# vgteam/vg

Hardware: AMD Instinct MI355X
Metric: reads/sec aligned (150 bp) (higher is better)
Workload: dtype u16

## Files before the change

### vg_amd/csrc/backend_hip.hip

```cpp
#include <chrono>
#include <thread>
#include <hip/hip_runtime.h>
#include <cstdlib>
#include <string>
#include "backend.hpp"
#include "pack_hip.hpp"

namespace vgk {

static __device__ __forceinline__ uint32_t from_lane_above(uint32_t x) {
    return (uint32_t)__builtin_amdgcn_update_dpp(0, (int)x, 0x138 , 0xf, 0xf, true);
}

template <int K>
struct TbStage {
    static constexpr uint32_t REC = (K + 3) / 4, RB = REC - 4;
    static constexpr uint32_t DWORDS = TB_TILE * 64u * REC;
    uint32_t* lds;
    __device__ __forceinline__ uint32_t* slot_a(uint32_t t, uint32_t lane) const { const uint32_t s = t % TB_TILE; return lds + (s * 64u + (lane ^ s)) * 4u; }
    __device__ __forceinline__ uint32_t* slot_b(uint32_t t, uint32_t lane) const { return lds + TB_TILE * 64u * 4u + ((t % TB_TILE) * 64u + lane) * RB; }
    __device__ __forceinline__ void flush(uint32_t* tile, uint32_t lane) const {
        __builtin_amdgcn_fence(__ATOMIC_ACQ_REL, "wavefront");
        __builtin_amdgcn_wave_barrier();
#pragma unroll
// ... 43 lines not shown
#pragma unroll
        for (int d = 32; d > 0; d >>= 1) { const uint32_t o = (uint32_t)__shfl_xor((int)shortest, d, 64); shortest = o < shortest ? o : shortest; }
        steady_steps(wd.G, shortest, wd.n_steps, steady_from, steady_to);
        steady_from = (uint32_t)__builtin_amdgcn_readfirstlane((int)steady_from); steady_to = (uint32_t)__builtin_amdgcn_readfirstlane((int)steady_to);
    }
    if constexpr (!CODES) {
        uint32_t t = 0;
        for (; t < steady_from; ++t) {
            if ((t & 3u) == 0) lane_prefetch(s, P, t);
            const uint32_t rh = from_lane_above(s.out_h), rf = from_lane_above(s.out_f), ri = from_lane_above(s.info);
            lane_step<K, S8, false, KEY3>(s, P, t, rh, rf, ri, nullptr, nullptr);
        }
        for (; t < steady_to; ++t) {
            if ((t & 3u) == 0) lane_prefetch(s, P, t);
            const uint32_t rh = from_lane_above(s.out_h), rf = from_lane_above(s.out_f), ri = from_lane_above(s.info);
            lane_step<K, S8, false, KEY3, false, true>(s, P, t, rh, rf, ri, nullptr, nullptr);
        }
        for (; t < wd.n_steps; ++t) {
            if ((t & 3u) == 0) lane_prefetch(s, P, t);
            const uint32_t rh = from_lane_above(s.out_h), rf = from_lane_above(s.out_f), ri = from_lane_above(s.info);
            lane_step<K, S8, false, KEY3>(s, P, t, rh, rf, ri, nullptr, nullptr);
        }
    }
    for (uint32_t t = 0; CODES && t < wd.n_steps; ++t) {
        if ((t & 3u) == 0) lane_prefetch(s, P, t);
        const uint32_t rh = from_lane_above(s.out_h);
        const uint32_t rf = from_lane_above(s.out_f);
        const uint32_t ri = from_lane_above(s.info);
        if constexpr (!CODES) {
        } else if constexpr (REWALK) {
            lane_step<K, S8, false>(s, P, t, rh, rf, ri, nullptr, nullptr);
            if (tb) {
                uint32_t* st = stage_lds[threadIdx.x >> 6] + lane * (TB_BND_CHUNK * 2u);
                const uint32_t slot = (t ^ lane) & (TB_BND_CHUNK - 1u);
                *reinterpret_cast<uint2*>(st + slot * 2u) = make_uint2(s.out_h, s.out_f);
                if ((t & (TB_BND_CHUNK - 1u)) == TB_BND_CHUNK - 1u || t + 1u == wd.n_steps) {
                    __builtin_amdgcn_fence(__ATOMIC_ACQ_REL, "wavefront"); __builtin_amdgcn_wave_barrier();
                    uint4* out = reinterpret_cast<uint4*>(tb + tb_bnd(wd.tb_off, wd.n_steps, t & ~(TB_BND_CHUNK - 1u), lane));
#pragma unroll
                    for (uint32_t j = 0; j < TB_BND_CHUNK; j += 2) {
                        const uint2 a = *reinterpret_cast<const uint2*>(st + ((j ^ lane) & (TB_BND_CHUNK - 1u)) * 2u), b = *reinterpret_cast<const uint2*>(st + (((j + 1u) ^ lane) & (TB_BND_CHUNK - 1u)) * 2u);
                        out[j >> 1] = make_uint4(a.x, a.y, b.x, b.y);
                    }
                    __builtin_amdgcn_fence(__ATOMIC_ACQ_REL, "wavefront"); __builtin_amdgcn_wave_barrier();
                }
                lane_store_checkpoint<K>(s, P, wd, t, lane);
            }
        } else if constexpr (TB_TILE > 1) {
            lane_step<K, S8, true, false, NOKEY>(s, P, t, rh, rf, ri, tb ? stage.slot_a(t, lane) : nullptr, stage.slot_b(t, lane));
            if (tb && ((t % TB_TILE) == TB_TILE - 1u || t + 1u == wd.n_steps)) stage.flush(tb + tb_tile_base(wd.tb_off, t, REC), lane);
        } else
            lane_step<K, S8, true, false, NOKEY>(s, P, t, rh, rf, ri, tb ? tb + tb_dword(wd.tb_off, t, lane, REC, 0) : nullptr, tb ? tb + tb_dword(wd.tb_off, t, lane, REC, 4) : nullptr);
    }
    if constexpr (NOKEY) return;
    if (REWALK || !CODES || !P.fused) {
#pragma unroll
        for (int half = 0; half < 2; ++half) {
            uint32_t prob; unsigned long long key;
            if (lane_best(s, half, prob, key)) atomicMax(&P.best[prob], key);
        }
        return;
    }
    unsigned long long* mine = reinterpret_cast<unsigned long long*>(stage_lds[threadIdx.x >> 6]);
#pragma unroll
    for (int half = 0; half < 2; ++half) {
        uint32_t prob; unsigned long long key = 0;
        if (!lane_best(s, half, prob, key)) key = 0;
        mine[lane * 2 + half] = key;
    }
    __threadfence();
    const uint32_t n_slots = 2u * (64u / wd.G);
    for (uint32_t slot = lane; slot < n_slots; slot += 64u) {
        const uint32_t q = slot >> 1, half = slot & 1u;
        if (wd.first_pair + q >= wd.pair_end) continue;
        const uint32_t prob = P.order[2u * (wd.first_pair + q) + half];
        if (prob == 0xffffffffu) continue;
        unsigned long long key = 0;
        for (uint32_t g = 0; g < wd.G; ++g) { const unsigned long long k = mine[(q * wd.G + g) * 2 + half]; key = k > key ? k : key; }
        walk_one(P, prob, key);
    }
}

#ifndef VGK_WALK_WAVES
#define VGK_WALK_WAVES 0
#endif
#if VGK_WALK_WAVES
__global__ __launch_bounds__(256, VGK_WALK_WAVES) void gssw_walk_kernel(const GsswParams P, const int in_fill_order) {
#else
__global__ __launch_bounds__(256) void gssw_walk_kernel(const GsswParams P, const int in_fill_order) {
#endif
    const uint32_t k = blockIdx.x * blockDim.x + threadIdx.x;
    if (!in_fill_order) { if (k < P.n_problems) walk_one(P, k, P.best[k]); return; }
    if (k >= 2u * P.n_pairs) return;
    const uint32_t i = P.order[k];
    if (i != 0xffffffffu) walk_one(P, i, P.best[i]);
}
__global__ __launch_bounds__(64) void banded_geometry_kernel(const BGeomParams P) {
    const uint32_t i = blockIdx.x * blockDim.x + threadIdx.x;
    if (i < P.n) banded_geometry_one(P, i);
}

__global__ __launch_bounds__(64) void gssw_walk_first_kernel(const GsswParams P, const int in_fill_order) {
    __shared__ uint32_t blk[2 * WD_DWORDS * 64];
    __shared__ int16_t tab[WD_TAB];
    if (threadIdx.x < WD_TAB) tab[threadIdx.x] = wd_table_entry(P, threadIdx.x);
    __syncthreads();
    const uint32_t k = blockIdx.x * blockDim.x + threadIdx.x;
    if (!in_fill_order) { if (k < P.n_problems) walk_first_one(P, k, P.best[k], blk + threadIdx.x, 64, tab); return; }
    if (k >= 2u * P.n_pairs) return;
    const uint32_t i = P.order[k];
    if (i != 0xffffffffu) walk_first_one(P, i, P.best[i], blk + threadIdx.x, 64, tab);
}
__global__ __launch_bounds__(64) void gssw_refill_layout_kernel(const GsswParams P) {
    refill_layout_one(P, blockIdx.x * blockDim.x + threadIdx.x);
}
__global__ __launch_bounds__(256) void gssw_refill_restore_kernel(const GsswParams P) {
    const uint32_t i = blockIdx.x * blockDim.x + threadIdx.x;
    if (i < P.n_problems) refill_restore_one(P, i);
}
__global__ __launch_bounds__(256) void gssw_walk_missed_kernel(const GsswParams P) {
    const uint32_t k = blockIdx.x * blockDim.x + threadIdx.x;
    if (k >= *tb_miss_count(P)) return;
    const uint32_t i = tb_miss_list(P)[k];
    walk_one(P, i, P.best[i]);
}

template <int K, bool S8>
__global__ __launch_bounds__(256, 2) void gssw_band_kernel(const GsswParams P) {
    const uint32_t wave = P.wave_begin + blockIdx.x * 4u + (threadIdx.x >> 6);
    if (wave >= P.wave_begin + P.wave_count) return;
    band_fill_lane<K, S8>(P, P.waves[wave], threadIdx.x & 63u);
}
__global__ __launch_bounds__(256) void gssw_bandwalk_kernel(const GsswParams P) {
    const uint32_t k = blockIdx.x * blockDim.x + threadIdx.x;
    if (k >= 2u * P.n_pairs) return;
    const uint32_t i = P.order[k];
    if (i != 0xffffffffu) bandwalk_one(P, i, P.best[i]);
}
template <int K, bool S8>
__global__ __launch_bounds__(64, 2) void gssw_rewalk_kernel(const GsswParams P) {
    __shared__ uint32_t win[(TB_CKPT / 2) * ((K + 3) / 4) * 64];
    const uint32_t count = *tb_miss_count(P);
    const uint32_t* list = tb_miss_list(P);
    for (uint32_t k = blockIdx.x * 64u + threadIdx.x; k < count; k += gridDim.x * 64u) {
        const uint32_t i = list[k];
        rewalk_one<K, S8>(P, i, P.best[i], win + threadIdx.x, 64u);
    }
}

static __device__ __forceinline__ uint32_t ops_of(const vgk_result* res, uint32_t i, uint32_t n) {
    return (i < n && res[i].status == VGK_OK) ? res[i].n_ops : 0u;
}
__global__ __launch_bounds__(256) void ops_scan_kernel(const vgk_result* res, uint32_t n, uint32_t* offs, uint32_t* sums) {
    __shared__ uint32_t wave_total[4];
    const uint32_t i0 = (blockIdx.x * 256u + threadIdx.x) * 4u, lane = threadIdx.x & 63u, w = threadIdx.x >> 6;
    const uint32_t c0 = ops_of(res, i0, n), c1 = ops_of(res, i0 + 1, n), c2 = ops_of(res, i0 + 2, n), c3 = ops_of(res, i0 + 3, n);
    uint32_t incl = c0 + c1 + c2 + c3;
#pragma unroll
    for (uint32_t d = 1; d < 64; d <<= 1) { const uint32_t up = __shfl_up(incl, d, 64); if (lane >= d) incl += up; }
    if (lane == 63) wave_total[w] = incl;
    __syncthreads();
    uint32_t before = 0;
    for (uint32_t k = 0; k < w; ++k) before += wave_total[k];
    uint32_t at = before + incl - (c0 + c1 + c2 + c3);
// ... 886 lines not shown
        return hipMemsetAsync(dst, 0, bytes, stream) == hipSuccess ? VGK_OK : VGK_ENODEV;
    }
    int sync() override {
        hipSetDevice(dev);
        return hipStreamSynchronize(stream) == hipSuccess ? VGK_OK : VGK_ENODEV;
    }
    size_t win_tmp_bytes(uint32_t n, uint32_t n_waves_cap) override { hipSetDevice(dev); return hip_win_tmp_bytes(n, n_waves_cap); }
    int win_stage1(const WinParams& P, void* tmp, size_t tmp_bytes) override { hipSetDevice(dev); return hip_win_stage1(P, tmp, tmp_bytes, copy); }
    int win_stage2(const WinParams& P, void* tmp, size_t tmp_bytes) override { hipSetDevice(dev); return hip_win_stage2(P, tmp, tmp_bytes, copy); }
    int download_side(void* dst, const void* src, size_t bytes) override {
        hipSetDevice(dev);
        if (hipMemcpyAsync(dst, src, bytes, hipMemcpyDeviceToHost, copy) != hipSuccess) return VGK_ENODEV;
        return hipStreamSynchronize(copy) == hipSuccess ? VGK_OK : VGK_ENODEV;
    }
    int fill_side(void* dst, int byte, size_t bytes) override {
        hipSetDevice(dev);
        return hipMemsetAsync(dst, byte, bytes, copy) == hipSuccess ? VGK_OK : VGK_ENODEV;
    }
    template <int K> int launch_fill_k(const GsswParams& p, hipStream_t stream) {
        const dim3 grid((p.wave_count + 3) / 4), block(256);
        const bool s8 = p.scale == 8, re = p.tb_mode == TB_REWALK;
        if (p.spec_fill == 1) {
            if (s8 && p.key3) hipLaunchKernelGGL((gssw_fill_kernel<K, true, false, false, true>), grid, block, 0, stream, p);
            else if (s8) hipLaunchKernelGGL((gssw_fill_kernel<K, true, false, false>), grid, block, 0, stream, p); else hipLaunchKernelGGL((gssw_fill_kernel<K, false, false, false>), grid, block, 0, stream, p);
            return VGK_OK;
        }
        if (p.spec_fill == 2 && s8 && !re && !p.fused) { hipLaunchKernelGGL((gssw_fill_kernel<K, true, false, true, false, true>), grid, block, 0, stream, p); return VGK_OK; }
        if (re) { if (s8) hipLaunchKernelGGL((gssw_fill_kernel<K, true, true>), grid, block, 0, stream, p); else hipLaunchKernelGGL((gssw_fill_kernel<K, false, true>), grid, block, 0, stream, p); }
        else    { if (s8) hipLaunchKernelGGL((gssw_fill_kernel<K, true, false>), grid, block, 0, stream, p); else hipLaunchKernelGGL((gssw_fill_kernel<K, false, false>), grid, block, 0, stream, p); }
        return VGK_OK;
    }
    int launch_fill(const GsswParams& p, hipStream_t stream) {
        switch (p.K) {
            case 16: return launch_fill_k<16>(p, stream);
            case 19: return launch_fill_k<19>(p, stream);
            case 20: return launch_fill_k<20>(p, stream);
            case 24: return launch_fill_k<24>(p, stream);
            default: return VGK_EINVAL;
        }
    }
    template <int K> void launch_rewalk_k(const GsswParams& p, hipStream_t stream) {
        const dim3 grid(1024), block(64);
        if (p.scale == 8) hipLaunchKernelGGL((gssw_rewalk_kernel<K, true>), grid, block, 0, stream, p); else hipLaunchKernelGGL((gssw_rewalk_kernel<K, false>), grid, block, 0, stream, p);
    }
    template <int K> void launch_band_k(const GsswParams& p, hipStream_t stream) {
        const dim3 grid((p.wave_count + 3) / 4), block(256);
        if (p.scale == 8) hipLaunchKernelGGL((gssw_band_kernel<K, true>), grid, block, 0, stream, p); else hipLaunchKernelGGL((gssw_band_kernel<K, false>), grid, block, 0, stream, p);
    }
    void launch_walk(const GsswParams& p0, const FillLaunch* launches, uint32_t n, hipStream_t stream, int lane = 0) {
        sev_set[lane] = false;
        if (p0.tb_mode != TB_REWALK) {
            if (p0.walk_passes == 2) {
                hipLaunchKernelGGL(gssw_walk_first_kernel, dim3((2 * p0.n_pairs + 63) / 64), dim3(64), 0, stream, p0, walk_in_fill_order ? 1 : 0);
                if (p0.spec_fill) {
                    const uint32_t max_waves = (p0.n_pairs + 64u / p0.refill_G - 1u) / (64u / p0.refill_G);
                    for (int k = 0; k < 2; ++k) if (!sev[lane][k]) hipEventCreate(&sev[lane][k]);
                    hipEventRecord(sev[lane][0], stream);
                    hipLaunchKernelGGL(gssw_refill_layout_kernel, dim3((max_waves + 63) / 64), dim3(64), 0, stream, p0);
                    GsswParams p = p0;
                    p.spec_fill = 2; p.K = p0.refill_K; p.wave_begin = p0.refill_wave0; p.wave_count = max_waves; p.wave_limit = p0.refill_count;
                    launch_fill(p, stream);
                    hipEventRecord(sev[lane][1], stream); sev_set[lane] = true;
                }
                hipLaunchKernelGGL(gssw_walk_missed_kernel, dim3((p0.n_problems + 255) / 256), dim3(256), 0, stream, p0);
            } else hipLaunchKernelGGL(gssw_walk_kernel, dim3((2 * p0.n_pairs + 255) / 256), dim3(256), 0, stream, p0, walk_in_fill_order ? 1 : 0);
            return;
        }
        GsswParams p = p0;
        for (uint32_t i = 0; i < n; ++i) {
            if (!launches[i].wave_count) continue;
            p.K = launches[i].K; p.wave_begin = launches[i].wave_begin; p.wave_count = launches[i].wave_count;
            switch (p.K) { case 16: launch_band_k<16>(p, stream); break; case 19: launch_band_k<19>(p, stream); break; case 20: launch_band_k<20>(p, stream); break; case 24: launch_band_k<24>(p, stream); break; default: break; }
        }
        hipLaunchKernelGGL(gssw_bandwalk_kernel, dim3((2 * p0.n_pairs + 255) / 256), dim3(256), 0, stream, p0);
        for (uint32_t i = 0; i < n; ++i) {
            if (!launches[i].wave_count) continue;
            p.K = launches[i].K; p.wave_begin = launches[i].wave_begin; p.wave_count = launches[i].wave_count;
            switch (p.K) { case 16: launch_rewalk_k<16>(p, stream); break; case 19: launch_rewalk_k<19>(p, stream); break; case 20: launch_rewalk_k<20>(p, stream); break; case 24: launch_rewalk_k<24>(p, stream); break; default: break; }
        }
    }
    int run_gssw(const GsswParams& p0, const FillLaunch* launches, uint32_t n, bool walk) override {
        hipSetDevice(dev);
        n_launches = n ? (int)n : 1;
        if (p0.n_problems == 0 || n == 0) { ms_fill = ms_walk = 0; pending = false; return VGK_OK; }
        GsswParams p = p0;
        if (p0.restore_probs) hipLaunchKernelGGL(gssw_refill_restore_kernel, dim3((p0.n_problems + 255) / 256), dim3(256), 0, stream, p0);
        if (fills_take_turns && fill_done_set[1]) hipStreamWaitEvent(stream, fill_done[1], 0);
        hipEventRecord(ev[0], stream);
        for (uint32_t i = 0; i < n; ++i) {
            const FillLaunch& L = launches[i];
            p.K = L.K; p.wave_begin = L.wave_begin; p.wave_count = L.wave_count;
            if (L.wave_count == 0) continue;
            hipStream_t st = (i == 0 || i > 2) ? stream : side[i - 1];
            if (st != stream) hipStreamWaitEvent(st, ev[0], 0);
            int rc = launch_fill(p, st);
            if (rc) return rc;
            if (st != stream) { hipEventRecord(side_done[i - 1], st); hipStreamWaitEvent(stream, side_done[i - 1], 0); }
        }
        hipEventRecord(ev[1], stream);
        hipEventRecord(fill_done[0], stream); fill_done_set[0] = true;
        timed_walk = walk && (!p.fused || p.tb_mode == TB_REWALK);
        if (timed_walk) {
            launch_walk(p0, launches, n, stream);
            hipEventRecord(ev[2], stream);
        }
        pending = true;
        return hipGetLastError() == hipSuccess ? VGK_OK : VGK_ENODEV;
    }
    int run_gssw_on(int lane, const GsswParams& p0, const FillLaunch* launches, uint32_t n, bool walk, void* done) override {
        hipSetDevice(dev);
        if (lane != 1 || n != 1 || p0.n_problems == 0) {
            if (lane == 1) lane1_on_main = true;
            if (hipMemsetAsync(p0.best, 0, ((size_t)p0.n_problems + 1) * sizeof(unsigned long long), stream) != hipSuccess) return VGK_ENODEV;
            int rc = run_gssw(p0, launches, n, walk);
            if (!rc && done) rc = hipEventRecord((hipEvent_t)done, stream) == hipSuccess ? VGK_OK : VGK_ENODEV;
            return rc;
        }
// ... 426 lines not shown
```

### vg_amd/csrc/gssw_device.hpp

```cpp
#pragma once
#include <stdint.h>
#include "../../include/vgk.h"
#include "pk16.hpp"

namespace vgk {

constexpr int KMAX = 24;

constexpr uint32_t XOFF = 1023;

enum : uint32_t {
    CI_BASE_MASK  = 7,
    CI_NODE_START = 8,
    CI_STORE_END  = 16,
    CI_SEED_SLOW  = 32,
    CI_INVALID    = 128
};
constexpr uint32_t CI_INVALID2 = CI_INVALID | (CI_INVALID << 16);

struct ProbDesc {
    uint32_t col_off;
    uint32_t R;
    uint32_t L;
    uint32_t read_off;
// ... 9 lines not shown
    uint32_t lane0;
    uint32_t geom;
    uint32_t Lpad;
    uint32_t bonus_start, bonus_end;
    uint32_t prof_off;
    uint32_t pad;
};

struct NodeRec {
    uint32_t col_start;
    uint32_t col_end;
    uint32_t pred_begin;
    uint32_t n_pred;
    int32_t  slot;
    uint32_t pinning;
};

struct WaveDesc {
    uint64_t tb_off;
    uint32_t n_steps;
    uint32_t first_pair;
    uint32_t G;
    uint32_t pair_end;
};

struct GsswParams {
    const ProbDesc* probs;
    const uint8_t*  colinfo;
    const uint8_t*  reads;
    const uint32_t* prof;
    const NodeRec*  nodes;
    const uint32_t* preds;
    uint32_t*       scratch;
    uint32_t*       tb;
    const WaveDesc* waves;
    const uint32_t* order;
    unsigned long long* best;
    vgk_result*     results;
    vgk_op*         ops;
    uint32_t n_problems, n_pairs, n_waves;
    uint32_t wave_begin, wave_count;
    uint32_t K;
    uint32_t prof4[6];
    uint32_t bias;
    uint32_t go, ge;
    int32_t  bonus;
    int32_t  want_tb;
    int32_t  spec_fill;
    uint32_t key3;
    int32_t  restore_probs;
    uint32_t refill_wave0, refill_pair0, refill_G, refill_K;
    unsigned long long refill_slot;
    uint32_t* refill_count;
    const uint32_t* wave_limit;
    int32_t  walk_passes;
    int32_t  tb_mode;
    int32_t  dbg;
    int32_t  fused;
    uint32_t scale;
    uint32_t xoff;
    int8_t   matrix[25];
};

VGK_HD uint32_t rep2(uint32_t x) { return (x & 0xffffu) * 0x00010001u; }

struct ProfWords {
    uint32_t w0, w1, w2, w3, w4;
    VGK_HD uint32_t of(uint32_t q) const {
        uint32_t a = w0, b = w1, c = w2, e = w3, f = w4;
#if defined(__HIP_DEVICE_COMPILE__)
        asm volatile("" : "+v"(a), "+v"(b), "+v"(c), "+v"(e), "+v"(f));
#endif
        uint32_t w = a; w = q == 1 ? b : w; w = q == 2 ? c : w; w = q == 3 ? e : w; w = q == 4 ? f : w;
        return w;
    }
    VGK_HD uint32_t of_row(uint32_t q) const { return q == 5 ? 0u : of(q); }
};
VGK_HD ProfWords prof_words(const GsswParams& P) { return ProfWords{P.prof4[0], P.prof4[1], P.prof4[2], P.prof4[3], P.prof4[4]}; }

VGK_HD uint32_t row_bonus(uint32_t bonus_start, uint32_t bonus_end, uint32_t row, uint32_t L) {
    return (row == 0 ? bonus_start : 0u) + (row + 1 == L ? bonus_end : 0u);
}

VGK_HD unsigned long long key64(uint32_t score, uint32_t col, uint32_t row) {
    return ((unsigned long long)score << 40) | ((unsigned long long)(0xFFFFFu - col) << 20) | (unsigned long long)(0xFFFFFu - row);
}

#ifndef VGK_PB_LDS
#define VGK_PB_LDS 0
#endif
template <int K>
struct Lane {
    uint32_t H[K];
    uint32_t E[K];
    uint32_t PA[K];
#if VGK_PB_LDS && defined(__HIPCC__)
    typedef __attribute__((address_space(3))) uint32_t lds_u32;
    lds_u32* PBL;
    VGK_HD uint32_t pb(int m) const { return *(const volatile lds_u32*)(PBL + 64 * m); }
    VGK_HD void set_pb(int m, uint32_t v) { PBL[64 * m] = v; }
#else
    uint32_t PB[K];
    VGK_HD uint32_t pb(int m) const { return PB[m]; }
    VGK_HD void set_pb(int m, uint32_t v) { PB[m] = v; }
#endif
    uint32_t out_h, out_f, info;
    uint32_t prev_rh;
    uint32_t best_lo, best_hi, step_lo, step_hi;
    uint32_t nodeA, nodeB;
    uint32_t g;
    uint32_t Lpad;
    uint32_t probA, probB;
    uint32_t LA, LB, flagsA, flagsB;
    uint32_t bsA, beA, bsB, beB;
    uint32_t RA, RB, colA, colB;
// ... 471 lines not shown
                const NodeRec& nr = nodes[node];
                if (xdrop && nr.n_pred == 0) {
                    if (r > 0) VGK_PUSH(node, VGK_OP_I, (uint32_t)r);
                    at_root = true; break;
                }
                int32_t found = -1;
                if (nr.n_pred == 1) found = (int32_t)P.preds[nr.pred_begin];
                else for (uint32_t k = 0; k < nr.n_pred; ++k) {
                    const uint32_t p = P.preds[nr.pred_begin + k];
                    if (w.saved_e(nodes[p], (uint32_t)r) == cur) { found = (int32_t)p; break; } }
                if (found < 0) { status = VGK_EINVAL; break; }
                pnode = (uint32_t)found; pc = nodes[pnode].col_end - 1; node_start = nodes[pnode].col_start;
            }
            const uint32_t fe = w.code((uint32_t)r, pc);
            if (fe & W_MISS) { status = W_MISSED; break; }
            if (!(fe & 4u)) { st = ST_H; cur += go; } else cur += ge;
            c = pc; node = pnode;
        } else {
            VGK_PUSH(node, VGK_OP_I, 1);
            if (r == 0) { status = VGK_EINVAL; break; }
            const uint32_t ff = w.code((uint32_t)r - 1, c);
            if (ff & W_MISS) { status = W_MISSED; break; }
            if (!(ff & 8u)) { st = ST_H; cur += go; } else cur += ge;
            r -= 1;
        }
    }
    if (xdrop && status == VGK_OK && !at_root) status = VGK_EINVAL;
    if (!xdrop && status == VGK_OK && r >= 0) VGK_PUSH(node, VGK_OP_S, (uint32_t)r + 1);
    if (status == VGK_OK) VGK_FLUSH();
#undef VGK_PUSH
#undef VGK_FLUSH
    res.status = status;
    if (status == VGK_OK) {
        res.n_ops = d.ops_cap - pos; res.ops_begin = d.ops_off + pos;
        res.first_offset = (int32_t)(first_c - node_start);
    }
    P.results[i] = res;
    return status;
}

VGK_HD void walk_one(const GsswParams& P, uint32_t i, unsigned long long best_key) {
    const ProbDesc d = P.probs[i];
    Walker w{P, d, (d.geom >> 16) & 1u, d.lane0, d.geom & 0xffu, P.waves[d.wave].tb_off, 0u, 0xffffffffu, 0u, 0xffffffffu};
    walk_body(P, i, d, w, best_key);
}

constexpr uint32_t WD_STEPS = 160, WD_DWORDS = WD_STEPS / 4;
struct alignas(16) WdQuad { uint32_t x, y, z, w; };
constexpr uint32_t WD_TAB = 40;
VGK_HD int16_t wd_table_entry(const GsswParams& P, uint32_t t) {
    const uint32_t q = t >> 3, b = t & 7u;
    return b < 4u ? (int16_t)((int32_t)((P.prof4[q] >> (8u * b)) & 0xffu) - (int32_t)P.bias) : (int16_t)0;
}
VGK_HD int32_t walk_diag_one(const GsswParams& P, uint32_t i, unsigned long long best_key, uint32_t* blk, uint32_t stride, const int16_t* tab) {
    const ProbDesc d = P.probs[i];
    const uint32_t mode = d.flags & 15u;
    if (mode != VGK_GSSW_LOCAL || d.prof_off != 0xffffffffu || d.L > WD_STEPS) return W_MISSED;
    const int32_t S = (int32_t)P.scale;
    const NodeRec* nodes = P.nodes + d.node_off;
    int32_t cur = 0; uint32_t c = 0, node = 0; int32_t r = 0;
    const bool have = walk_end_cell(P, d, best_key, [&](const NodeRec&, uint32_t) { return 0u; }, cur, c, node, r);
    if (have && cur >= 2047 * S) return W_MISSED;
    vgk_result res;
    res.score = 0; res.status = VGK_OK; res.end_node = -1; res.end_offset = -1; res.end_read = -1; res.first_offset = 0; res.n_ops = 0; res.ops_begin = d.ops_off;
    if (!have || cur <= 0) { P.results[i] = res; return VGK_OK; }
    const uint32_t r_at = d.read_off + (uint32_t)r, c_at = d.col_off + c;
    if (r_at + 1u < WD_STEPS || c_at + 1u < WD_STEPS) return W_MISSED;
    { const uint8_t* rsrc = P.reads + (r_at + 1u - WD_STEPS); const uint8_t* csrc = P.colinfo + (c_at + 1u - WD_STEPS);
      WdQuad rq[WD_DWORDS / 4], cq[WD_DWORDS / 4];
      for (uint32_t j = 0; j < WD_DWORDS / 4; ++j) { __builtin_memcpy(&rq[j], rsrc + 16u * j, 16); __builtin_memcpy(&cq[j], csrc + 16u * j, 16); }
      for (uint32_t j = 0; j < WD_DWORDS / 4; ++j) {
          blk[(4u * j + 0u) * stride] = rq[j].x; blk[(4u * j + 1u) * stride] = rq[j].y; blk[(4u * j + 2u) * stride] = rq[j].z; blk[(4u * j + 3u) * stride] = rq[j].w;
          blk[(WD_DWORDS + 4u * j + 0u) * stride] = cq[j].x; blk[(WD_DWORDS + 4u * j + 1u) * stride] = cq[j].y; blk[(WD_DWORDS + 4u * j + 2u) * stride] = cq[j].z; blk[(WD_DWORDS + 4u * j + 3u) * stride] = cq[j].w;
      } }
    const uint32_t end_start = nodes[node].col_start;
    res.score = cur / S; res.end_node = (int32_t)node; res.end_offset = (int32_t)(c - end_start); res.end_read = r;
    if (!(d.flags & VGK_GSSW_TRACEBACK)) { P.results[i] = res; return VGK_OK; }
    vgk_op* ops = P.ops + d.ops_off;
    uint32_t pos = d.ops_cap;
    bool room_ok = true;
    auto put = [&](uint32_t nd, uint32_t op, uint32_t len) { if (pos == 0) { room_ok = false; return; } --pos; ops[pos].node = nd; ops[pos].len = (uint16_t)len; ops[pos].op = (uint8_t)op; ops[pos].pad = 0; };
    if (r < (int32_t)d.L - 1) put(node, VGK_OP_S, d.L - 1 - (uint32_t)r);
    int32_t v = cur - (r + 1 == (int32_t)d.L ? (int32_t)d.bonus_end : 0);
    uint32_t run_node = node, run_from = 0, taken = 0;
    int verdict = 0;
    uint32_t n_it = (uint32_t)r + 1u < c + 1u ? (uint32_t)r + 1u : c + 1u;
    n_it = n_it < WD_STEPS ? n_it : WD_STEPS;
    uint32_t rw = 0, cw = 0;
    bool fresh = true;
    uint32_t col_base = c;
    for (uint32_t k = 0; k < n_it; ++k) {
        const uint32_t at = WD_STEPS - 1u - k;
        if ((at & 3u) == 3u || fresh) { rw = blk[(at >> 2) * stride]; cw = blk[(WD_DWORDS + (at >> 2)) * stride]; fresh = false; }
        const uint32_t ci = (cw >> (8u * (at & 3u))) & 0xffu, q = (rw >> (8u * (at & 3u))) & 0xffu;
        v -= (int32_t)tab[8u * q + (ci & CI_BASE_MASK)] + (k == (uint32_t)r ? (int32_t)d.bonus_start : 0);
        ++taken;
        if (v <= 0) { verdict = v == 0 ? 1 : -1; break; }
        if (ci & CI_NODE_START) {
            if (!(ci & CI_SEED_SLOW) && run_node != 0u) {
                put(run_node, VGK_OP_M, taken - run_from); run_node -= 1u; run_from = taken;
                continue;
            }
            const uint32_t row = (uint32_t)r - k;
            if (row == 0u || k + 1u >= WD_STEPS) { verdict = -1; break; }
            const NodeRec nr = nodes[run_node];
            int32_t found = -1;
            if (nr.n_pred == 1u) found = (int32_t)P.preds[nr.pred_begin];
            else for (uint32_t kk = 0; kk < nr.n_pred; ++kk) {
                const uint32_t p = P.preds[nr.pred_begin + kk];
                const int32_t slot = nodes[p].slot;
                if (slot >= 0 && (int32_t)(P.scratch[d.scratch_off + (uint32_t)slot * d.Lpad + (row - 1u)] & 0xffffu) == v) { found = (int32_t)p; break; }
            }
            if (found < 0) { verdict = -1; break; }
            const uint32_t pc = nodes[found].col_end - 1u, c_abs = d.col_off + pc, next_at = WD_STEPS - 2u - k;
            if (c_abs < next_at) { verdict = -1; break; }
            put(run_node, VGK_OP_M, taken - run_from); run_node = (uint32_t)found; run_from = taken;
            const uint8_t* csrc = P.colinfo + (c_abs - next_at);
            for (uint32_t j = 0; 4u * j <= next_at; ++j) {
                uint32_t w; __builtin_memcpy(&w, csrc + 4u * j, 4);
                blk[(WD_DWORDS + j) * stride] = w;
            }
            fresh = true; col_base = pc + k + 1u;
            const uint32_t more = row < pc + 1u ? row : pc + 1u;
            n_it = k + 1u + more < WD_STEPS ? k + 1u + more : WD_STEPS;
        }
    }
    const uint32_t run_len = taken - run_from;
    if (verdict != 1 || !room_ok) return W_MISSED;
    put(run_node, VGK_OP_M, run_len);
    const int32_t r_left = r - (int32_t)taken;
    if (r_left >= 0) put(run_node, VGK_OP_S, (uint32_t)r_left + 1u);
    if (!room_ok) return W_MISSED;
    const uint32_t first_c = col_base - (taken - 1u);
    res.n_ops = d.ops_cap - pos; res.ops_begin = d.ops_off + pos;
    res.first_offset = (int32_t)(first_c - nodes[run_node].col_start);
    P.results[i] = res;
    return VGK_OK;
}
VGK_HD uint32_t* tb_miss_count(const GsswParams& P);
VGK_HD void tb_miss_add(const GsswParams& P, uint32_t i);
VGK_HD void walk_first_one(const GsswParams& P, uint32_t i, unsigned long long best_key, uint32_t* blk, uint32_t stride, const int16_t* tab) {
    if (walk_diag_one(P, i, best_key, blk, stride, tab) == W_MISSED) tb_miss_add(P, i);
}

enum : int32_t { TB_CODES = 0, TB_REWALK = 1 };
constexpr uint32_t TB_CKPT = 16;

constexpr uint32_t TB_SLACK = 8;
VGK_HD uint32_t tb_band_cols(uint32_t K) { return K + 2u * TB_SLACK + TB_CKPT - 1u; }
struct TbBand { uint32_t cs, hi; bool used; };
VGK_HD TbBand tb_band_of(uint32_t r_e, uint32_t c_e, uint32_t g, uint32_t K) {
    TbBand b; b.used = g * K <= r_e; b.cs = 0; b.hi = 0;
    if (!b.used) return b;
    const uint32_t r_hi = g * K + K - 1u < r_e ? g * K + K - 1u : r_e;
    const uint32_t back_lo = r_e - g * K + TB_SLACK, back_hi = r_e - r_hi;
    const uint32_t lo = c_e > back_lo ? c_e - back_lo : 0u;
    uint32_t hi = c_e > back_hi ? c_e - back_hi + TB_SLACK : TB_SLACK;
    if (hi > c_e) hi = c_e;
    b.cs = lo / TB_CKPT * TB_CKPT;
    const uint32_t last = b.cs + tb_band_cols(K) - 1u;
    b.hi = hi < last ? hi : last;
    return b;
}

constexpr uint32_t TB_BND_CHUNK = 16;
VGK_HD uint32_t tb_steps_padded(uint32_t n_steps) { return (n_steps + TB_BND_CHUNK - 1u) / TB_BND_CHUNK * TB_BND_CHUNK; }
VGK_HD uint64_t tb_bnd_dwords(uint32_t n_steps) { return 128ull * tb_steps_padded(n_steps); }

VGK_HD uint64_t tb_wave_dwords(uint32_t n_steps, uint32_t K) {
    const uint64_t rec = (K + 3u) >> 2;
    const uint64_t codes = (uint64_t)((n_steps + TB_TILE - 1) / TB_TILE * TB_TILE) * 64u * rec;
    const uint64_t rewalk = tb_bnd_dwords(n_steps) + (uint64_t)((n_steps + TB_CKPT - 1) / TB_CKPT) * 128u * K + 64ull * tb_band_cols(K) * rec;
    return codes > rewalk ? codes : rewalk;
}
VGK_HD uint64_t tb_bnd(uint64_t tb_off, uint32_t n_steps, uint32_t t, uint32_t lane) { return tb_off + ((uint64_t)lane * tb_steps_padded(n_steps) + t) * 2u; }
VGK_HD uint64_t tb_ckpt(uint64_t tb_off, uint32_t n_steps, uint32_t cb, uint32_t lane, uint32_t K) {
    return tb_off + tb_bnd_dwords(n_steps) + ((uint64_t)cb * 64u + lane) * 2u * K;
}
VGK_HD uint64_t tb_band(uint64_t tb_off, uint32_t n_steps, uint32_t x, uint32_t lane, uint32_t K) {
    return tb_off + tb_bnd_dwords(n_steps) + (uint64_t)((n_steps + TB_CKPT - 1) / TB_CKPT) * 128u * K + ((uint64_t)x * 64u + lane) * ((K + 3u) >> 2);
}

template <int K>
VGK_HD void lane_store_boundary(const Lane<K>& s, const GsswParams& P, const WaveDesc& wd, uint32_t t, uint32_t lane) {
    uint32_t* b = P.tb + tb_bnd(wd.tb_off, wd.n_steps, t, lane);
    b[0] = s.out_h; b[1] = s.out_f;
}
template <int K>
VGK_HD void lane_store_checkpoint(const Lane<K>& s, const GsswParams& P, const WaveDesc& wd, uint32_t t, uint32_t lane) {
    const uint32_t c = t - s.g;
    if (t >= s.g && (c & (TB_CKPT - 1u)) == TB_CKPT - 1u && !((s.info & CI_INVALID) && (s.info & (CI_INVALID << 16)))) {
// ... 268 lines not shown
```

### vg_amd/csrc/vgk_api.cpp

```cpp
#include <algorithm>
#include <chrono>
#include <cstdio>
#include <cstdlib>
#include <cstring>
#include <memory>
#include <mutex>
#include <new>
#include <string>
#include <vector>
#include "backend.hpp"
#include "ctx.hpp"
#include "host_parallel.hpp"

#include "batch.hpp"
#include "gssw_wide.hpp"

extern "C" {

int vgk_abi_version(void) { return VGK_ABI_VERSION; }

const char* vgk_strerror(int code) {
    switch (code) {
        case VGK_OK: return "ok";
        case VGK_EINVAL: return "invalid argument";
// ... 344 lines not shown
        if (launches.empty() || launches.back().K != K) launches.push_back(FillLaunch{K, n_waves, 0});
        n_pairs = bk.pair1; n_waves += (bk.pair1 - bk.pair0 + gpw - 1) / gpw;
        launches.back().wave_count = n_waves - launches.back().wave_begin;
        buckets.push_back(bk);
        s0 = s1;
    }
    uint32_t local_tb = 0;
    for (uint32_t i = 0; i < n; ++i) local_tb += (problems[i].flags & (15u | VGK_GSSW_TRACEBACK)) == (uint32_t)(VGK_GSSW_LOCAL | VGK_GSSW_TRACEBACK) ? 1u : 0u;
    const bool fused_env = std::getenv("VGAMD_FUSED_TRACEBACK") && std::atoi(std::getenv("VGAMD_FUSED_TRACEBACK"));
    const bool walk2 = !fused_env && n >= 1024 && 2ull * local_tb >= n && !std::getenv("VGAMD_WALK_ONE_PASS");
    bool spec = walk2 && b->want_tb && buckets.size() == 1 && launches.size() == 1 && default_tb_mode(fused_env ? 1 : 0, !all.far) == TB_CODES && !std::getenv("VGAMD_NO_SPEC_FILL");
    uint64_t refill_slot = 0;
    if (spec) { uint32_t rmax_all = 0; for (uint32_t i = 0; i < n; ++i) rmax_all = std::max(rmax_all, probs[i].R);
                refill_slot = tb_wave_dwords(rmax_all + buckets[0].G - 1, buckets[0].K); }
    std::vector<uint32_t> order((size_t)(spec ? 4 : 2) * n_pairs, 0xffffffffu);
    std::vector<WaveDesc> waves((size_t)(spec ? 2 : 1) * n_waves);
    parallel_for(n_waves, [&](uint32_t w, unsigned) {
        size_t bi = 0;
        while (bi + 1 < buckets.size() && buckets[bi + 1].wave0 <= w) ++bi;
        const Bucket& bk = buckets[bi];
        const uint32_t gpw = 64 / bk.G, pw = bk.pair0 + (w - bk.wave0) * gpw;
        WaveDesc wd{};
        wd.first_pair = pw; wd.G = bk.G; wd.pair_end = bk.pair1;
        uint32_t rmax = 0;
        for (uint32_t q = 0; q < gpw && pw + q < bk.pair1; ++q)
            for (uint32_t h = 0; h < 2; ++h) {
                const uint32_t k = bk.s0 + 2 * (pw + q - bk.pair0) + h;
                const uint32_t i = k < bk.s1 ? idx[k] : 0xffffffffu;
                order[2 * (size_t)(pw + q) + h] = i;
                if (i == 0xffffffffu) continue;
                rmax = std::max(rmax, probs[i].R);
                probs[i].wave = w; probs[i].lane0 = q * bk.G; probs[i].geom = bk.K | (bk.G << 8) | (h << 16);
            }
        wd.n_steps = rmax ? rmax + bk.G - 1 : 0;
        wd.tb_off = b->want_tb ? tb_wave_dwords(wd.n_steps, bk.K) : 0;
        waves[w] = wd;
    });
    uint64_t tb_dwords = 0;
    for (uint32_t w = 0; w < n_waves; ++w) { WaveDesc& wd = waves[w]; const uint64_t size = wd.tb_off; wd.tb_off = tb_dwords; tb_dwords += size; b->wave_steps += wd.n_steps; }
    if (spec && (uint64_t)n_waves * refill_slot > tb_dwords + tb_dwords / 2) spec = false;
    if (spec) tb_dwords = (uint64_t)n_waves * refill_slot;

    lap("waves");
    lk.lock();
    if ((rc = to_device(b, (const ProbDesc*)probs, (size_t)n, P.probs))) return fail(rc);
    if ((rc = to_device(b, waves, P.waves))) return fail(rc);
    if ((rc = to_device(b, order, P.order, 2))) return fail(rc);
    if ((rc = dev_alloc(b, (size_t)scratch_words + 16, P.scratch))) return fail(rc);
    if ((rc = dev_alloc(b, (size_t)tb_dwords + 4, P.tb))) return fail(rc);
    if ((rc = dev_alloc(b, (size_t)tb_best_entries(n), P.best))) return fail(rc);
    if ((rc = dev_alloc(b, (size_t)n + 1, P.results))) return fail(rc);
    if ((rc = dev_alloc(b, (size_t)ops_total + 1, P.ops))) return fail(rc);
    P.spec_fill = 0; P.wave_limit = nullptr; P.refill_count = nullptr; P.refill_wave0 = P.refill_pair0 = P.refill_G = P.refill_K = 0; P.refill_slot = 0;
    if (spec) {
        if ((rc = dev_alloc(b, (size_t)4, P.refill_count))) return fail(rc);
        P.spec_fill = 1; P.refill_wave0 = n_waves; P.refill_pair0 = n_pairs; P.refill_G = buckets[0].G; P.refill_K = buckets[0].K; P.refill_slot = refill_slot;
    }
    lap("allocs");
    lk.unlock();
    if ((rc = issue_uploads())) return fail(rc);
    P.wave_begin = 0; P.wave_count = 0; P.K = 0;
    P.n_problems = n; P.n_pairs = n_pairs; P.n_waves = n_waves;
    const uint32_t S = ctx->scale;
    for (int q = 0; q < 6; ++q) P.prof4[q] = ctx->prof4[q] * S;
    P.bias = ctx->bias * S; P.go = ctx->sc.gap_open * S; P.ge = ctx->sc.gap_extend * S; P.bonus = ctx->sc.full_length_bonus * (int32_t)S;
    P.scale = S; P.xoff = XOFF * S;
    P.want_tb = b->want_tb ? 1 : 0;
    P.fused = 0;
    if (const char* e = std::getenv("VGAMD_FUSED_TRACEBACK")) P.fused = std::atoi(e) ? 1 : 0;
    P.dbg = std::getenv("VGAMD_TB_DBG") ? std::atoi(std::getenv("VGAMD_TB_DBG")) : 0; P.tb_mode = default_tb_mode(P.fused, !all.far);
    P.walk_passes = walk2 && !P.fused ? 2 : 1;
    if (P.walk_passes != 2 || P.tb_mode != TB_CODES) P.spec_fill = 0;
    P.key3 = 0;
    if (P.spec_fill) {
        uint32_t longest = 0; bool xdrop = false;
        for (uint32_t i = 0; i < n; ++i) { longest = std::max(longest, probs[i].L); xdrop = xdrop || (problems[i].flags & 15u) == (uint32_t)VGK_XDROP_PINNED; }
        P.key3 = gssw_key3_ok(S, ctx->has_qa, xdrop, longest, (uint32_t)std::max(0, ctx->max_score), (uint32_t)std::max(0, ctx->max_bonus)) && !std::getenv("VGAMD_NO_KEY3") ? 1u : 0u;
    }
    std::memcpy(P.matrix, ctx->sc.matrix, 25);
    b->ops_total = ops_total;
    if ((rc = ctx->be->sync_side())) return fail(rc);
    lap("uploads");
    *out = hb.release();
    return VGK_OK;
} catch (const std::bad_alloc&) { return VGK_ENOMEM; } catch (...) { return VGK_EINVAL; }

static void observe_speculation(vgk_batch* b) {
    if (!b->ran || !b->ran_spec || b->spec_observed || !b->P.refill_count) return;
    b->spec_observed = true;
    uint32_t refilled = 0;
    if (b->ctx->be->download_fetch(&refilled, b->P.refill_count, sizeof refilled) != VGK_OK) return;
    b->ctx->spec.observe(b->P.n_waves ? (double)refilled / (double)b->P.n_waves : 0.0, b->spec_probe);
}

int vgk_gssw_run(vgk_batch* b) try {
    if (!b) return VGK_EINVAL;
    std::lock_guard<std::mutex> lk(b->ctx->mu);
    if (!b->done) b->done = b->ctx->be->event_create();
    GsswParams P = b->P;
    if (b->P.spec_fill) {
        if (b->ran && b->ran_spec && !b->spec_observed && b->ctx->be->event_done(b->done)) observe_speculation(b);
        bool probe = false;
        const bool speculate = b->ctx->spec.decide(&probe);
        b->spec_probe = probe;
        if (!speculate) {
            P.spec_fill = 0; P.wave_limit = nullptr;
// ... 244 lines not shown
```

### vg_amd/csrc/window_api.cpp

```cpp
#include <algorithm>
#include <atomic>
#include <chrono>
#include <cstdio>
#include <cstdlib>
#include <cstring>
#include <memory>
#include <mutex>
#include <new>
#include <vector>
#include "batch.hpp"
#include "dgraph.hpp"
#include "host_parallel.hpp"


namespace {

inline int ref_code(char ch) {
    switch (ch) { case 'A': return 0; case 'C': return 1; case 'G': return 2; case 'T': return 3; default: return 4; }
}

struct Lap {
    std::chrono::steady_clock::time_point t0 = std::chrono::steady_clock::now(); const bool on = std::getenv("VGAMD_TIMING") != nullptr;
    void operator()(const char* what) {
        if (!on) return;
// ... 197 lines not shown
    lap("problems staged");
    if ((rc = be->win_stage1(W, tmp, tmp_bytes))) return fail(rc);
    if (!on_device && (rc = staged_upload(0, (void*)W.raw_reads, reads, reads_bytes))) return fail(rc);
    lap("reads staged");
    WinTotals T;
    if ((rc = be->download_side(&T, W.totals, sizeof T))) return fail(rc);
    lap("stage 1 (sizes)");
    if (T.first_bad != ~0ull) return fail(-(int)(T.first_bad & 0xffu));
    for (uint32_t k = 0; k < WIN_COLS; ++k) if (T.tot[k] >= (1ull << 32)) return fail(VGK_ETOOBIG);
    if (extensions && n) {
        uint32_t* st_nodes = (uint32_t*)lease.s->get(4, (ext_nodes_total + 1) * 4); uint32_t* st_count = (uint32_t*)lease.s->get(6, (uint64_t)n * 4);
        if (!st_nodes || !st_count) return fail(VGK_ENOMEM);
        if ((rc = be->download_side(st_count, W.ext_count, (size_t)n * 4))) return fail(rc);
        if ((rc = be->download_side(st_nodes, W.kept_node, (size_t)ext_nodes_total * 4))) return fail(rc);
        b->ext_count.assign(st_count, st_count + n); b->ext_nodes.assign(st_nodes, st_nodes + ext_nodes_total);
        b->ext_off.resize((size_t)n + 1);
        for (uint32_t i = 0; i < n; ++i) b->ext_off[i] = extensions[i].kept_off;
        b->ext_off[n] = (uint32_t)ext_nodes_total;
        lap("extension nodes");
    }
    b->want_tb = T.want_tb != 0; b->cells = T.cells; b->tb_cells = T.tb_cells; b->in_bytes = T.in_bytes;
    W.want_tb = b->want_tb ? 1 : 0;
    uint8_t* colinfo; uint8_t* rd; NodeRec* nodes; uint32_t* preds; WaveDesc* waves; uint32_t* order;
    {
        std::lock_guard<std::mutex> lk(ctx->mu);
        colinfo = (uint8_t*)take_keep(T.tot[WS_COLS] + 8); rd = (uint8_t*)take_keep(T.tot[WS_READS] + 8);
        nodes = (NodeRec*)take_keep((T.tot[WS_NODES] + 1) * sizeof(NodeRec)); preds = (uint32_t*)take_keep((T.tot[WS_PREDS] + 1) * 4);
        waves = (WaveDesc*)take_keep((uint64_t)waves_cap * sizeof(WaveDesc)); order = (uint32_t*)take_keep(((uint64_t)waves_cap * 4 + 4) * 4);
        rc = dev_alloc(b, (size_t)T.tot[WS_SCRATCH] + 16, P.scratch);
        if (!rc) rc = dev_alloc(b, (size_t)tb_best_entries(n), P.best);
        if (!rc) rc = dev_alloc(b, (size_t)n + 1, P.results);
        if (!rc) rc = dev_alloc(b, (size_t)T.tot[WS_OPS] + 1, P.ops);
        if (!rc && (!colinfo || !rd || !nodes || !preds || !waves || !order)) rc = VGK_ENOMEM;
    }
    if (rc) return fail(rc);
    W.colinfo = colinfo; W.reads = rd; W.nodes = nodes; W.preds = preds; W.waves = waves; W.order = order;
    if ((rc = be->fill_side(colinfo + T.tot[WS_COLS], (int)CI_INVALID, 8))) return fail(rc);
    if ((rc = be->win_stage2(W, tmp, tmp_bytes))) return fail(rc);
    if ((rc = be->download_side(&T, W.totals, sizeof T))) return fail(rc);
    lap("stage 2 (order, waves, arenas)");
    if (T.n_waves > waves_cap || T.n_launches > 4) return fail(VGK_EINVAL);
    uint32_t local_tb = 0;
    if (!on_device) for (uint32_t i = 0; i < n; ++i) local_tb += (problems[i].flags & (15u | VGK_GSSW_TRACEBACK)) == (uint32_t)(VGK_GSSW_LOCAL | VGK_GSSW_TRACEBACK) ? 1u : 0u;
    const bool walk2 = !on_device && n >= 1024 && 2ull * local_tb >= n && !std::getenv("VGAMD_WALK_ONE_PASS");
    bool spec = walk2 && b->want_tb && T.n_launches == 1 && T.n_buckets == 1 && T.first_G && default_tb_mode(0, near_chain) == TB_CODES && 2ull * T.n_waves <= waves_cap &&
                !std::getenv("VGAMD_NO_SPEC_FILL");
    uint64_t refill_slot = 0, tb_dwords = T.tb_dwords;
    if (spec) {
        refill_slot = tb_wave_dwords(T.max_steps, T.launch_K[0]);
        if ((uint64_t)T.n_waves * refill_slot > T.tb_dwords + T.tb_dwords / 2) spec = false;
        else tb_dwords = (uint64_t)T.n_waves * refill_slot;
    }
    P.spec_fill = 0; P.wave_limit = nullptr; P.refill_count = nullptr; P.refill_wave0 = P.refill_pair0 = P.refill_G = P.refill_K = 0; P.refill_slot = 0;
    {
        std::lock_guard<std::mutex> lk(ctx->mu);
        rc = dev_alloc(b, (size_t)tb_dwords + 4, P.tb);
        if (!rc && spec) rc = dev_alloc(b, (size_t)4, P.refill_count);
    }
    if (rc) return fail(rc);
    if (spec) { P.spec_fill = 1; P.refill_wave0 = T.n_waves; P.refill_pair0 = T.n_pairs; P.refill_G = T.first_G; P.refill_K = T.launch_K[0]; P.refill_slot = refill_slot; }
    for (uint32_t k = 0; k < T.n_launches; ++k) b->launches.push_back(FillLaunch{T.launch_K[k], T.launch_begin[k], T.launch_count[k]});
    P.probs = W.probs; P.colinfo = colinfo; P.reads = rd; P.prof = nullptr; P.nodes = nodes; P.preds = preds; P.waves = waves; P.order = order;
    P.wave_begin = 0; P.wave_count = 0; P.K = 0;
    P.n_problems = n; P.n_pairs = T.n_pairs; P.n_waves = T.n_waves;
    const uint32_t S = ctx->scale;
    for (int q = 0; q < 6; ++q) P.prof4[q] = ctx->prof4[q] * S;
    P.bias = ctx->bias * S; P.go = ctx->sc.gap_open * S; P.ge = ctx->sc.gap_extend * S; P.bonus = ctx->sc.full_length_bonus * (int32_t)S;
    P.scale = S; P.xoff = XOFF * S;
    P.want_tb = b->want_tb ? 1 : 0;
    P.fused = 0; P.dbg = std::getenv("VGAMD_TB_DBG") ? std::atoi(std::getenv("VGAMD_TB_DBG")) : 0; P.tb_mode = default_tb_mode(0, near_chain);
    P.walk_passes = walk2 ? 2 : 1;
    if (P.walk_passes != 2 || P.tb_mode != TB_CODES) P.spec_fill = 0;
    P.key3 = 0;
    if (P.spec_fill) {
        uint32_t longest = 0; bool xdrop = false;
        for (uint32_t i = 0; i < n; ++i) { longest = std::max(longest, problems[i].read_len); xdrop = xdrop || (problems[i].flags & 15u) == (uint32_t)VGK_XDROP_PINNED; }
        P.key3 = gssw_key3_ok(S, ctx->has_qa, xdrop, longest, (uint32_t)std::max(0, ctx->max_score), (uint32_t)std::max(0, ctx->max_bonus)) && !std::getenv("VGAMD_NO_KEY3") ? 1u : 0u;
    }
    std::memcpy(P.matrix, ctx->sc.matrix, 25);
    b->ops_total = T.tot[WS_OPS]; b->wave_steps = T.wave_steps;
    lap("done");
    *out = hb.release();
    return VGK_OK;
} catch (const std::bad_alloc&) { return VGK_ENOMEM; } catch (...) { return VGK_EINVAL; }

int vgk_gssw_pack_windows(vgk_ctx* ctx, const vgk_dgraph* dg, const char* reads, size_t reads_bytes,
                          const vgk_window_problem* problems, uint32_t n, uint32_t ops_per_problem, vgk_batch** out) try {
    return vgk_pack_windows_impl(ctx, dg, reads, reads_bytes, problems, n, ops_per_problem, out, false, 0, nullptr);
} catch (const std::bad_alloc&) { return VGK_ENOMEM; } catch (...) { return VGK_EINVAL; }

int vgk_gssw_pack_extensions(vgk_ctx* ctx, const vgk_dgraph* dg, const char* reads, size_t reads_bytes,
                             const vgk_extension_problem* problems, uint32_t n, uint32_t ops_per_problem, vgk_batch** out) try {
    if (!ctx || !dg || dg->ctx != ctx || !out || (!problems && n) || (!reads && reads_bytes)) return VGK_EINVAL;
    if (!dg->g.succ_off) return VGK_EUNSUPPORTED;
    std::vector<vgk_window_problem> win(n); std::vector<WinExt> ext(n);
    uint64_t at = 0;
    for (uint32_t i = 0; i < n; ++i) {
        const vgk_extension_problem& p = problems[i];
        vgk_window_problem& w = win[i]; WinExt& x = ext[i];
        w.read_off = p.read_off; w.read_len = p.read_len; w.flags = p.flags; w.first_node = p.first_node; w.n_nodes = p.n_nodes; w.max_gap_length = p.max_gap_length; w.reserved = 0;
        x.start_node = p.start_node; x.start_offset = p.start_offset; x.query_offset = p.query_offset; x.leftward = p.leftward ? 1u : 0u; x.kept_off = (uint32_t)at; x.pad = 0;
        at += p.n_nodes;
        if (at >= (1ull << 32) - 16) return VGK_ETOOBIG;
    }
    return vgk_pack_windows_impl(ctx, dg, reads, reads_bytes, win.data(), n, ops_per_problem, out, false, 0, ext.data());
} catch (const std::bad_alloc&) { return VGK_ENOMEM; } catch (...) { return VGK_EINVAL; }
// ... 3 lines not shown
```

Baseline: 69.13 million.

## Stage walk-first tiles cooperatively per wave and optionally fuse missed walk into refill

```diff
diff --git a/vg_amd/csrc/backend_hip.hip b/vg_amd/csrc/backend_hip.hip
--- a/vg_amd/csrc/backend_hip.hip
+++ b/vg_amd/csrc/backend_hip.hip
@@ -119,7 +119,18 @@
         } else
             lane_step<K, S8, true, false, NOKEY>(s, P, t, rh, rf, ri, tb ? tb + tb_dword(wd.tb_off, t, lane, REC, 0) : nullptr, tb ? tb + tb_dword(wd.tb_off, t, lane, REC, 4) : nullptr);
     }
-    if constexpr (NOKEY) return;
+    if constexpr (NOKEY) {
+        if (!P.refill_walk) return;
+        __threadfence();
+        const uint32_t n_slots = 2u * (64u / wd.G);
+        for (uint32_t slot = lane; slot < n_slots; slot += 64u) {
+            const uint32_t q = slot >> 1, half = slot & 1u;
+            if (wd.first_pair + q >= wd.pair_end) continue;
+            const uint32_t prob = P.order[2u * (wd.first_pair + q) + half];
+            if (prob != 0xffffffffu) walk_one(P, prob, P.best[prob]);
+        }
+        return;
+    }
     if (REWALK || !CODES || !P.fused) {
 #pragma unroll
         for (int half = 0; half < 2; ++half) {
@@ -167,16 +178,46 @@
     if (i < P.n) banded_geometry_one(P, i);
 }
 
+#ifndef VGK_WD_COOP
+#define VGK_WD_COOP 1
+#endif
+constexpr uint32_t WD_LDS_STRIDE = VGK_WD_COOP ? 65u : 64u, WD_TURNS = 16u;
 __global__ __launch_bounds__(64) void gssw_walk_first_kernel(const GsswParams P, const int in_fill_order) {
-    __shared__ uint32_t blk[2 * WD_DWORDS * 64];
+    __shared__ uint32_t blk[2 * WD_DWORDS * WD_LDS_STRIDE];
     __shared__ int16_t tab[WD_TAB];
     if (threadIdx.x < WD_TAB) tab[threadIdx.x] = wd_table_entry(P, threadIdx.x);
+    const uint32_t lane = threadIdx.x, k = blockIdx.x * blockDim.x + threadIdx.x;
+    uint32_t i = 0xffffffffu;
+    if (!in_fill_order) { if (k < P.n_problems) i = k; }
+    else if (k < 2u * P.n_pairs) i = P.order[k];
+    WdStart w; w.roff = 0; w.coff = 0;
+    int32_t st = VGK_OK;
+    if (i != 0xffffffffu) st = wd_start(P, i, P.best[i], w);
+    const bool go = i != 0xffffffffu && st == WD_RUN;
+#if VGK_WD_COOP
+    const unsigned long long mask = __ballot(go);
+    if (mask) {
+        const int first = __builtin_amdgcn_readfirstlane(__ffsll((long long)mask) - 1);
+        const uint32_t ro = go ? w.roff : (uint32_t)__shfl((int)w.roff, first, 64), co = go ? w.coff : (uint32_t)__shfl((int)w.coff, first, 64);
+        if (lane < WD_DWORDS) {
+            for (uint32_t n0 = 0; n0 < 64u; n0 += WD_TURNS) {
+                uint32_t a[WD_TURNS], b[WD_TURNS];
+#pragma unroll
+                for (uint32_t n = 0; n < WD_TURNS; ++n) {
+                    const uint32_t rn = (uint32_t)__builtin_amdgcn_readlane((int)ro, (int)(n0 + n)), cn = (uint32_t)__builtin_amdgcn_readlane((int)co, (int)(n0 + n));
+                    __builtin_memcpy(&a[n], P.reads + rn + 4u * lane, 4); __builtin_memcpy(&b[n], P.colinfo + cn + 4u * lane, 4);
+                }
+#pragma unroll
+                for (uint32_t n = 0; n < WD_TURNS; ++n) { blk[lane * WD_LDS_STRIDE + n0 + n] = a[n]; blk[(WD_DWORDS + lane) * WD_LDS_STRIDE + n0 + n] = b[n]; }
+            }
+        }
+    }
+#else
+    if (go) wd_stage_lane(P, w, blk + lane, WD_LDS_STRIDE);
+#endif
     __syncthreads();
-    const uint32_t k = blockIdx.x * blockDim.x + threadIdx.x;
-    if (!in_fill_order) { if (k < P.n_problems) walk_first_one(P, k, P.best[k], blk + threadIdx.x, 64, tab); return; }
-    if (k >= 2u * P.n_pairs) return;
-    const uint32_t i = P.order[k];
-    if (i != 0xffffffffu) walk_first_one(P, i, P.best[i], blk + threadIdx.x, 64, tab);
+    if (go) st = wd_run(P, i, w, blk + lane, WD_LDS_STRIDE, tab);
+    if (i != 0xffffffffu && st == W_MISSED) tb_miss_add(P, i);
 }
 __global__ __launch_bounds__(64) void gssw_refill_layout_kernel(const GsswParams P) {
     refill_layout_one(P, blockIdx.x * blockDim.x + threadIdx.x);
@@ -1169,17 +1210,20 @@
         if (p0.tb_mode != TB_REWALK) {
             if (p0.walk_passes == 2) {
                 hipLaunchKernelGGL(gssw_walk_first_kernel, dim3((2 * p0.n_pairs + 63) / 64), dim3(64), 0, stream, p0, walk_in_fill_order ? 1 : 0);
+                const bool own_walk = p0.spec_fill && p0.refill_walk && p0.scale == 8 && !p0.fused;
                 if (p0.spec_fill) {
                     const uint32_t max_waves = (p0.n_pairs + 64u / p0.refill_G - 1u) / (64u / p0.refill_G);
                     for (int k = 0; k < 2; ++k) if (!sev[lane][k]) hipEventCreate(&sev[lane][k]);
                     hipEventRecord(sev[lane][0], stream);
                     hipLaunchKernelGGL(gssw_refill_layout_kernel, dim3((max_waves + 63) / 64), dim3(64), 0, stream, p0);
                     GsswParams p = p0;
+                    p.refill_walk = own_walk ? 1 : 0;
                     p.spec_fill = 2; p.K = p0.refill_K; p.wave_begin = p0.refill_wave0; p.wave_count = max_waves; p.wave_limit = p0.refill_count;
                     launch_fill(p, stream);
                     hipEventRecord(sev[lane][1], stream); sev_set[lane] = true;
                 }
-                hipLaunchKernelGGL(gssw_walk_missed_kernel, dim3((p0.n_problems + 255) / 256), dim3(256), 0, stream, p0);
+                if (!own_walk)
+                    hipLaunchKernelGGL(gssw_walk_missed_kernel, dim3((p0.n_problems + 255) / 256), dim3(256), 0, stream, p0);
             } else hipLaunchKernelGGL(gssw_walk_kernel, dim3((2 * p0.n_pairs + 255) / 256), dim3(256), 0, stream, p0, walk_in_fill_order ? 1 : 0);
             return;
         }
diff --git a/vg_amd/csrc/gssw_device.hpp b/vg_amd/csrc/gssw_device.hpp
--- a/vg_amd/csrc/gssw_device.hpp
+++ b/vg_amd/csrc/gssw_device.hpp
@@ -85,6 +85,7 @@
     uint32_t refill_wave0, refill_pair0, refill_G, refill_K;
     unsigned long long refill_slot;
     uint32_t* refill_count;
+    int32_t  refill_walk;
     const uint32_t* wave_limit;
     int32_t  walk_passes;
     int32_t  tb_mode;
@@ -94,6 +95,8 @@
     uint32_t xoff;
     int8_t   matrix[25];
 };
+
+constexpr int32_t REFILL_WALK_DEFAULT = 0;
 
 VGK_HD uint32_t rep2(uint32_t x) { return (x & 0xffffu) * 0x00010001u; }
 
@@ -671,27 +674,44 @@
     const uint32_t q = t >> 3, b = t & 7u;
     return b < 4u ? (int16_t)((int32_t)((P.prof4[q] >> (8u * b)) & 0xffu) - (int32_t)P.bias) : (int16_t)0;
 }
-VGK_HD int32_t walk_diag_one(const GsswParams& P, uint32_t i, unsigned long long best_key, uint32_t* blk, uint32_t stride, const int16_t* tab) {
-    const ProbDesc d = P.probs[i];
+constexpr int32_t WD_RUN = 101;
+struct WdStart { ProbDesc d; int32_t cur; uint32_t c, node; int32_t r; uint32_t roff, coff; };
+VGK_HD int32_t wd_start(const GsswParams& P, uint32_t i, unsigned long long best_key, WdStart& w) {
+    w.d = P.probs[i];
+    const ProbDesc& d = w.d;
     const uint32_t mode = d.flags & 15u;
     if (mode != VGK_GSSW_LOCAL || d.prof_off != 0xffffffffu || d.L > WD_STEPS) return W_MISSED;
     const int32_t S = (int32_t)P.scale;
-    const NodeRec* nodes = P.nodes + d.node_off;
     int32_t cur = 0; uint32_t c = 0, node = 0; int32_t r = 0;
     const bool have = walk_end_cell(P, d, best_key, [&](const NodeRec&, uint32_t) { return 0u; }, cur, c, node, r);
     if (have && cur >= 2047 * S) return W_MISSED;
+    if (!have || cur <= 0) {
+        vgk_result res;
+        res.score = 0; res.status = VGK_OK; res.end_node = -1; res.end_offset = -1; res.end_read = -1; res.first_offset = 0; res.n_ops = 0; res.ops_begin = d.ops_off;
+        P.results[i] = res; return VGK_OK;
+    }
+    const uint32_t r_at = d.read_off + (uint32_t)r, c_at = d.col_off + c;
+    if (r_at + 1u < WD_STEPS || c_at + 1u < WD_STEPS) return W_MISSED;
+    w.cur = cur; w.c = c; w.node = node; w.r = r;
+    w.roff = r_at + 1u - WD_STEPS; w.coff = c_at + 1u - WD_STEPS;
+    return WD_RUN;
+}
+VGK_HD void wd_stage_lane(const GsswParams& P, const WdStart& w, uint32_t* blk, uint32_t stride) {
+    const uint8_t* rsrc = P.reads + w.roff; const uint8_t* csrc = P.colinfo + w.coff;
+    WdQuad rq[WD_DWORDS / 4], cq[WD_DWORDS / 4];
+    for (uint32_t j = 0; j < WD_DWORDS / 4; ++j) { __builtin_memcpy(&rq[j], rsrc + 16u * j, 16); __builtin_memcpy(&cq[j], csrc + 16u * j, 16); }
+    for (uint32_t j = 0; j < WD_DWORDS / 4; ++j) {
+        blk[(4u * j + 0u) * stride] = rq[j].x; blk[(4u * j + 1u) * stride] = rq[j].y; blk[(4u * j + 2u) * stride] = rq[j].z; blk[(4u * j + 3u) * stride] = rq[j].w;
+        blk[(WD_DWORDS + 4u * j + 0u) * stride] = cq[j].x; blk[(WD_DWORDS + 4u * j + 1u) * stride] = cq[j].y; blk[(WD_DWORDS + 4u * j + 2u) * stride] = cq[j].z; blk[(WD_DWORDS + 4u * j + 3u) * stride] = cq[j].w;
+    }
+}
+VGK_HD int32_t wd_run(const GsswParams& P, uint32_t i, const WdStart& w, uint32_t* blk, uint32_t stride, const int16_t* tab) {
+    const ProbDesc& d = w.d;
+    const int32_t S = (int32_t)P.scale;
+    const NodeRec* nodes = P.nodes + d.node_off;
+    const int32_t cur = w.cur; const uint32_t c = w.c, node = w.node; const int32_t r = w.r;
     vgk_result res;
     res.score = 0; res.status = VGK_OK; res.end_node = -1; res.end_offset = -1; res.end_read = -1; res.first_offset = 0; res.n_ops = 0; res.ops_begin = d.ops_off;
-    if (!have || cur <= 0) { P.results[i] = res; return VGK_OK; }
-    const uint32_t r_at = d.read_off + (uint32_t)r, c_at = d.col_off + c;
-    if (r_at + 1u < WD_STEPS || c_at + 1u < WD_STEPS) return W_MISSED;
-    { const uint8_t* rsrc = P.reads + (r_at + 1u - WD_STEPS); const uint8_t* csrc = P.colinfo + (c_at + 1u - WD_STEPS);
-      WdQuad rq[WD_DWORDS / 4], cq[WD_DWORDS / 4];
-      for (uint32_t j = 0; j < WD_DWORDS / 4; ++j) { __builtin_memcpy(&rq[j], rsrc + 16u * j, 16); __builtin_memcpy(&cq[j], csrc + 16u * j, 16); }
-      for (uint32_t j = 0; j < WD_DWORDS / 4; ++j) {
-          blk[(4u * j + 0u) * stride] = rq[j].x; blk[(4u * j + 1u) * stride] = rq[j].y; blk[(4u * j + 2u) * stride] = rq[j].z; blk[(4u * j + 3u) * stride] = rq[j].w;
-          blk[(WD_DWORDS + 4u * j + 0u) * stride] = cq[j].x; blk[(WD_DWORDS + 4u * j + 1u) * stride] = cq[j].y; blk[(WD_DWORDS + 4u * j + 2u) * stride] = cq[j].z; blk[(WD_DWORDS + 4u * j + 3u) * stride] = cq[j].w;
-      } }
     const uint32_t end_start = nodes[node].col_start;
     res.score = cur / S; res.end_node = (int32_t)node; res.end_offset = (int32_t)(c - end_start); res.end_read = r;
     if (!(d.flags & VGK_GSSW_TRACEBACK)) { P.results[i] = res; return VGK_OK; }
@@ -756,6 +776,13 @@
     P.results[i] = res;
     return VGK_OK;
 }
+VGK_HD int32_t walk_diag_one(const GsswParams& P, uint32_t i, unsigned long long best_key, uint32_t* blk, uint32_t stride, const int16_t* tab) {
+    WdStart w;
+    const int32_t st = wd_start(P, i, best_key, w);
+    if (st != WD_RUN) return st;
+    wd_stage_lane(P, w, blk, stride);
+    return wd_run(P, i, w, blk, stride, tab);
+}
 VGK_HD uint32_t* tb_miss_count(const GsswParams& P);
 VGK_HD void tb_miss_add(const GsswParams& P, uint32_t i);
 VGK_HD void walk_first_one(const GsswParams& P, uint32_t i, unsigned long long best_key, uint32_t* blk, uint32_t stride, const int16_t* tab) {
diff --git a/vg_amd/csrc/vgk_api.cpp b/vg_amd/csrc/vgk_api.cpp
--- a/vg_amd/csrc/vgk_api.cpp
+++ b/vg_amd/csrc/vgk_api.cpp
@@ -420,6 +420,7 @@
     if ((rc = dev_alloc(b, (size_t)n + 1, P.results))) return fail(rc);
     if ((rc = dev_alloc(b, (size_t)ops_total + 1, P.ops))) return fail(rc);
     P.spec_fill = 0; P.wave_limit = nullptr; P.refill_count = nullptr; P.refill_wave0 = P.refill_pair0 = P.refill_G = P.refill_K = 0; P.refill_slot = 0;
+    P.refill_walk = std::getenv("VGAMD_REFILL_WALK") ? (std::atoi(std::getenv("VGAMD_REFILL_WALK")) ? 1 : 0) : REFILL_WALK_DEFAULT;
     if (spec) {
         if ((rc = dev_alloc(b, (size_t)4, P.refill_count))) return fail(rc);
         P.spec_fill = 1; P.refill_wave0 = n_waves; P.refill_pair0 = n_pairs; P.refill_G = buckets[0].G; P.refill_K = buckets[0].K; P.refill_slot = refill_slot;
diff --git a/vg_amd/csrc/window_api.cpp b/vg_amd/csrc/window_api.cpp
--- a/vg_amd/csrc/window_api.cpp
+++ b/vg_amd/csrc/window_api.cpp
@@ -273,6 +273,7 @@
         else tb_dwords = (uint64_t)T.n_waves * refill_slot;
     }
     P.spec_fill = 0; P.wave_limit = nullptr; P.refill_count = nullptr; P.refill_wave0 = P.refill_pair0 = P.refill_G = P.refill_K = 0; P.refill_slot = 0;
+    P.refill_walk = std::getenv("VGAMD_REFILL_WALK") ? (std::atoi(std::getenv("VGAMD_REFILL_WALK")) ? 1 : 0) : REFILL_WALK_DEFAULT;
     {
         std::lock_guard<std::mutex> lk(ctx->mu);
         rc = dev_alloc(b, (size_t)tb_dwords + 4, P.tb);
```

Result: no change. 69.36 million (median of 6 runs) (+0.3%).
